# LouisBearing/BirdSoundClassif

Hardware: AMD Instinct MI355X
Metric: clips/sec (3 s @ 22.05 kHz) detect fwd (higher is better)
Workload: dtype f32

## Files before the change

birdsoundclassif_amd/_lib.py:

```python
import ctypes as C
import os
import subprocess

_HERE = os.path.dirname(os.path.abspath(__file__))
LIB_PATH = os.environ.get('NBM_LIB') or os.path.join(_HERE, 'libnbm_hip.so')
CSRC = os.path.join(_HERE, 'csrc')

_lib = None


class GemmDesc(C.Structure):
    _fields_ = [('x', C.c_void_p), ('w', C.c_void_p), ('y', C.c_void_p),
                ('scale', C.c_void_p), ('shift', C.c_void_p), ('residual', C.c_void_p),
                ('x_gs', C.c_int64), ('w_gs', C.c_int64), ('y_gs', C.c_int64), ('res_gs', C.c_int64),
                ('groups', C.c_int),
                ('B', C.c_int), ('H', C.c_int), ('W', C.c_int), ('Cin', C.c_int),
                ('N', C.c_int),
                ('kh', C.c_int), ('kw', C.c_int), ('stride', C.c_int), ('pad', C.c_int),
                ('Ho', C.c_int), ('Wo', C.c_int),
                ('x_ld', C.c_int), ('w_ld', C.c_int), ('y_ld', C.c_int), ('res_ld', C.c_int),
                ('alpha', C.c_float), ('act', C.c_int), ('shift_per_row', C.c_int),
                ('up', C.c_void_p), ('up_H', C.c_int), ('up_W', C.c_int),
                ('rows', C.c_void_p), ('rows_blocks', C.c_void_p),
                ('rows_mode', C.c_int), ('rows_count', C.c_int), ('rows_TH', C.c_int), ('rows_TW', C.c_int),
                ('mask', C.c_void_p), ('mask_ld', C.c_int), ('bits_out', C.c_void_p)]


class RoiDesc(C.Structure):
    _fields_ = [('fmap', C.c_void_p * 5), ('fh', C.c_int * 5), ('fw', C.c_int * 5),
                ('n_levels', C.c_int), ('C', C.c_int),
                ('rois', C.c_void_p), ('n_roi', C.c_void_p), ('B', C.c_int), ('roi_cap', C.c_int),
                ('pe_f', C.c_void_p), ('pe_t', C.c_void_p), ('img_h', C.c_int), ('img_w', C.c_int),
                ('pool', C.c_void_p), ('pe', C.c_void_p), ('level', C.c_void_p), ('n_roi_per_image', C.c_int)]


class AugmentParams(C.Structure):
    _fields_ = [('gain', C.c_float), ('coef', C.c_float), ('denom', C.c_float), ('neg_coef', C.c_float),
                ('neg_denom', C.c_float), ('flags', C.c_int32), ('hard_index', C.c_int32), ('pad', C.c_int32),
                ('noise_seed', C.c_uint64)]


class BwdDesc(C.Structure):
    _fields_ = [('g', C.c_void_p), ('w', C.c_void_p), ('x', C.c_void_p), ('out', C.c_void_p),
                ('a_scale', C.c_void_p), ('row_scale', C.c_void_p), ('residual', C.c_void_p), ('mask', C.c_void_p),
                ('g_gs', C.c_int64), ('w_gs', C.c_int64), ('x_gs', C.c_int64), ('out_gs', C.c_int64), ('res_gs', C.c_int64),
                ('groups', C.c_int),
                ('B', C.c_int), ('H', C.c_int), ('W', C.c_int), ('Cin', C.c_int), ('N', C.c_int),
                ('kh', C.c_int), ('kw', C.c_int), ('stride', C.c_int), ('pad', C.c_int), ('Ho', C.c_int), ('Wo', C.c_int),
                ('g_ld', C.c_int), ('w_ld', C.c_int), ('x_ld', C.c_int), ('out_ld', C.c_int), ('res_ld', C.c_int),
                ('mask_ld', C.c_int), ('alpha', C.c_float), ('bias_grad', C.c_void_p), ('residual2', C.c_void_p), ('res2_ld', C.c_int),
                ('mask_bits', C.c_void_p)]


_P, _I, _L, _F, _U64 = C.c_void_p, C.c_int, C.c_int64, C.c_float, C.c_uint64

SIGNATURES = {
    'nbm_graph_census': [_P, C.POINTER(C.c_longlong * 6)],
    'nbm_copy_rect': [_P, _P, _L, _L, _I, _L, _L, _I, _I, _P],
    'nbm_gemm_conv': [C.POINTER(GemmDesc), _P],
    'nbm_pcm16_to_wave': [_P, _L, _I, _I, _I, _P, _L, _L, _P, _L, _I, _I, _P],
    'nbm_resample_to_wave': [_P, _L, _I, _L, _I, _I, _P, _I, _L, _L, _P, _L, _I, _I, _I, _P],
    'nbm_minmax_init': [_P, _I, _P],
    'nbm_stft_db': [_P, _L, _I, _I, _I, _I, _P, _I, _I, _I, _F, _P, _L, _I, _P, _P],
    'nbm_spec_windows': [_P, _L, _I, _I, _I, _I, _P, _P, _I, _I, _I, _P, _P],
    'nbm_spec_windows_table': [_P, _I, _I, _P, _I, _I, _P],
    'nbm_init_conv': [_P, _L, _P, _P, _I, _P, _P],
    'nbm_stem7x7': [_P, _I, _I, _I, _P, _P, _P, _P, _P, _P, _P],
    'nbm_stem7x7_wgrad': [_P, _P, _I, _I, _I, _P, _P, _P],
    'nbm_maxpool3x3s2': [_P, _I, _I, _I, _I, _P, _I, _I, _P, _P],
    'nbm_space_to_batch2': [_P, _I, _I, _I, _I, _P, _I, _P],
    'nbm_avgpool2x2': [_P, _I, _I, _I, _I, _P, _P],
    'nbm_avgpool2x2_bwd': [_P, _I, _I, _I, _I, _P, _P],
    'nbm_upsample_bilinear_add': [_P, _I, _I, _I, _I, _P, _P, _I, _I, _P],
    'nbm_softmax_rows': [_P, _L, _I, _L, _P],
    'nbm_dwconv3x3': [_P, _I, _I, _I, _I, _I, _I, _P, _P, _P, _L, _P, _I, _I, _P],
    'nbm_silu': [_P, _P, _L, _P],
    'nbm_layernorm': [_P, _L, _I, _P, _P, _F, _P, _P],
    'nbm_mha_small': [_P, _P, _P, _I, _I, _I, _P, _I, _I, _I, _I, _I, _L, _L, _P, _F, _P],
    'nbm_pair_softmax': [_P, _L, _I, _I, _P, _I, _P],
    'nbm_rpn_decode': [_P, _P, _P, _I, _I, _I, _I, _I, _I, _P, _P, _P, _P],
    'nbm_rpn_select': [_P, _P, _P, _I, _I, _I, _I, _I, _P, _P, _P, _I, _P],
    'nbm_nms_batched': [_P, _P, _P, _I, _I, _F, _I, _P, _P, _P, _P, _P, _I, _P],
    'nbm_rpn_select_seg': [_P, _P, _P, _I, _I, _I, _I, _I, _P, _P, _P, _P, _P],
    'nbm_nms_batched_seg': [_P, _P, _P, _I, _I, _F, _I, _P, _P, _P, _P, _P, _P, _P],
    'nbm_roi_pool': [C.POINTER(RoiDesc), _P],
    'nbm_rcnn_post': [_P, _P, _I, _I, _P, _P, _I, _I, _I, _F, _F, _I, _P, _P, _I, _P],
    'nbm_merge_collect': [_P, _P, _I, _I, _I, _I, _I, _L, _P, _P, _P, _P, _P, _P],
    'nbm_merge_nms_workspace': [_I, C.POINTER(C.c_int64)],
    'nbm_merge_nms': [_P, _P, _I, _F, _P, _L, _P, _P, _P],
    'nbm_merge_gather': [_P, _P, _P, _P, _P, _I, _P, _P, _P],
    'nbm_conv_dgrad': [C.POINTER(BwdDesc), _P],
    'nbm_conv_wgrad': [C.POINTER(BwdDesc), _P],
    'nbm_relu_bwd': [_P, _P, _P, _L, _P],
    'nbm_silu_bwd': [_P, _P, _P, _L, _P],
    'nbm_axpby': [_P, _P, _P, _F, _F, _L, _L, _P],
    'nbm_colsum': [_P, _L, _I, _I, _P, _P],
    'nbm_leaky_relu_bwd': [_P, _P, _P, _F, _L, _P],
    'nbm_layernorm_bwd': [_P, _P, _P, _L, _I, _F, _P, _P, _P, _P],
    'nbm_mha_small_bwd': [_P, _P, _P, _P, _I, _I, _I, _I, _P, _P, _P, _I, _I, _I, _P, _I, _I, _I, _I, _L, _L, _P, _F, _P],
    'nbm_zero_roi_windows': [_P, _I, _I, _I, _P, _P, _I, _I, _I, _P],
    'nbm_zero_pattern': [_P, _I, _I, _I, _I, _I, _P],
    'nbm_zero_tiles': [_P, _I, _I, _I, _I, _P, _I, _P, _P],
    'nbm_tiles_gather': [_P, _I, _I, _I, _I, _P, _I, _P, _P, _P],
    'nbm_tiles_scatter_add': [_P, _I, _I, _I, _I, _P, _I, _P, _P, _P],
    'nbm_proposal_iou': [_P, _P, _P, _I, _I, _I, _P, _P, _P],
    'nbm_anchor_targets': [_P, _I, _P, _P, _I, _I, _F, _F, _P, _P, _P, _P],
    'nbm_maxpool3x3s2_bwd': [_P, _P, _P, _I, _I, _I, _I, _I, _I, _P, _P, _P],
    'nbm_upsample_bilinear_bwd': [_P, _I, _I, _I, _I, _P, _I, _I, _I, _P],
    'nbm_tiles_upsample_bilinear_bwd_add': [_P, _I, _I, _I, _I, _P, _I, _P, _P, _I, _I, _P],
    'nbm_png_unfilter_gray8': [_P, _L, _I, _I, _I, _P, _L, _P, _P],
    'nbm_image_half_std_u8': [_P, _L, _I, _L, _P, _P],
    'nbm_randn_fill': [_U64, _L, _P, _P],
    'nbm_augment_batch': [_P, _P, _P, _I, _I, _I, _P, _P, _P, _P, _P, _P, _P],
    'nbm_u8_to_unit': [_P, _L, _P, _P],
    'nbm_wino_input': [_P, _I, _I, _I, _I, _P, _I, _P],
    'nbm_wino_output': [_P, _P, _P, _P, _I, _I, _I, _I, _I, _P, _I, _P, _P],
    'nbm_wino_outgrad': [_P, _I, _I, _I, _I, _P, _P, _I, _P],
    'nbm_wino_weight': [_P, _P, _I, _I, _I, _I, _P, _P],
    'nbm_wino_weight_grad': [_P, _P, _I, _I, _I, _P, _P],
    'nbm_wino23_rows': [_P, _I, _I, _I, _I, _P, _P],
    'nbm_wino23_conv_fused': [_P, _P, _P, _P, _P, _I, _I, _I, _I, _I, _I, _P, _I, _P],
    'nbm_wino23_rows_tiles': [_P, _I, _I, _I, _I, _P, _I, _P, _P, _P, _I, _P],
    'nbm_wino23_conv_fused_tiles': [_P, _P, _P, _P, _P, _I, _I, _I, _I, _I, _I, _P, _P, _I, _P, _P, _P],
    'nbm_roi_tiles': [_P, _P, _I, _I, _I, _I, _P, _P, _P, _I, _P, _P, _I, _P],
    'nbm_wino23_input_tiles': [_P, _I, _I, _I, _I, _P, _I, _P, _P, _P],
    'nbm_wino23_outgrad_tiles': [_P, _I, _I, _I, _I, _P, _I, _P, _P, _P, _I, _P],
    'nbm_cell_outgrad': [_P, _I, _I, _I, _I, _I, _P, _P, _P],
    'nbm_cell_weight': [_P, _I, _I, _P, _I, _P, _I, _P],
    'nbm_cell_weight_fold': [_P, _P, _I, _I, _I, _I, _F, _P, _I, _P, _I, _P],
    'nbm_cell_weight_grad': [_P, _I, _I, _I, _P, _P],
    'nbm_cell_input': [_P, _I, _I, _I, _I, _I, _P, _I, _I, _P],
    'nbm_cell_input_up': [_P, _P, _I, _I, _I, _I, _I, _I, _I, _P, _I, _I, _P],
    'nbm_cell_patches': [_P, _I, _I, _I, _I, _I, _P, _I, _I, _P],
    'nbm_cell_patches_up': [_P, _P, _I, _I, _I, _I, _I, _I, _I, _P, _I, _I, _P],
    'nbm_cell_dgrad_output': [_P, _I, _I, _I, _I, _I, _P, _I, _I, _I, _P, _P],
    'nbm_cell_output': [_P, _P, _I, _I, _I, _I, _I, _P, _P],
    'nbm_weighted_sum': [_P, _P, _P, _P, _P, _L, _P],
    'nbm_weighted_sum_bwd': [_P, _P, _P, _P, _P, _P, _P, _P, _P, _L, _P],
    'nbm_softmax_rows_bwd': [_P, _P, _P, _L, _I, _F, _P],
    'nbm_pair_softmax_bwd': [_P, _P, _P, _L, _P],
    'nbm_dwconv3x3_bwd': [_P, _P, _P, _I, _I, _I, _I, _I, _I, _P, _P, _P, _I, _I, _P],
    'nbm_dwconv3x3_bwd_acc': [_P, _P, _I, _I, _I, _I, _I, _I, _P, _I, _I, _P],
    'nbm_film_fwd': [_P, _P, _P, _L, _I, _P],
    'nbm_film_bwd': [_P, _P, _P, _P, _P, _L, _I, _P],
    'nbm_bn_train_fwd': [_P, _L, _I, _P, _P, _F, _F, _P, _P, _P, _P, _P, _P, _P],
    'nbm_bn_train_bwd': [_P, _P, _L, _I, _P, _P, _P, _P, _P, _P, _P, _P],
    'nbm_roi_pool_bwd': [C.POINTER(C.c_void_p), C.POINTER(C.c_int), C.POINTER(C.c_int), _I, _I, _P, _P, _I, _I, _P, _P],
    'nbm_sqnorm_accum': [_P, _L, _P, _P],
    'nbm_adamw_step': [_P, _P, _P, _P, _L, _F, _F, _F, _F, _F, _I, _P, _F, _P],
}


def build(verbose=False):
    r = subprocess.run(['make', '-C', CSRC, '-j4'], capture_output=True, text=True)
    if verbose or r.returncode:
        print(r.stdout[-4000:], r.stderr[-4000:])
    if r.returncode:
        raise RuntimeError('building libnbm_hip.so failed')
    return LIB_PATH


def load():
    global _lib
    if _lib is not None:
        return _lib
    import torch
    if not os.path.isfile(LIB_PATH):
        raise RuntimeError(f'{LIB_PATH} is missing: build it with `python -c "import __graft_entry__ as g; g.build()"` '
                           '(the NBM hot path has no CPU / eager fallback)')
    lib = C.CDLL(LIB_PATH)
    lib.nbm_version.restype = C.c_char_p
    lib.nbm_version.argtypes = []
    for name, argtypes in SIGNATURES.items():
        fn = getattr(lib, name)
        fn.argtypes = argtypes
        fn.restype = C.c_int
    _lib = lib
    return lib


class NbmHipError(RuntimeError):
    pass


_CODES = {-1: 'NBM_EINVAL (bad argument / shape)', -2: 'NBM_EALIGN (pointer or pitch not 16-byte aligned)',
          -3: 'NBM_EUNSUPPORTED'}


def check(rc, name):
    if rc != 0:
        raise NbmHipError(f'{name} failed: {_CODES.get(rc, f"hipError_t {rc}")}')
```

birdsoundclassif_amd/nets/backbone.py:

```python
import torch
from torch import nn

from .. import ops
from . import _prep, functional as Fn
from .position_encoding import build_position_encoding

bcbk_channels = {'resnet': {'2': 64, '3': 256, '4': 512, '5': 1024, '6': 2048}}
_RESNET_LAYERS = {'resnet50': [3, 4, 6, 3], 'resnet101': [3, 4, 23, 3], 'resnet152': [3, 8, 36, 3]}


class FrozenBatchNorm2d(nn.Module):

    def __init__(self, n):
        super().__init__()
        self.register_buffer('weight', torch.ones(n))
        self.register_buffer('bias', torch.zeros(n))
        self.register_buffer('running_mean', torch.zeros(n))
        self.register_buffer('running_var', torch.ones(n))

    def _load_from_state_dict(self, state_dict, prefix, local_metadata, strict, missing_keys, unexpected_keys,
                              error_msgs):
        state_dict.pop(prefix + 'num_batches_tracked', None)
        super()._load_from_state_dict(state_dict, prefix, local_metadata, strict, missing_keys, unexpected_keys,
                                      error_msgs)

    def affine(self):
        return _prep.bn_affine(self.weight, self.bias, self.running_mean, self.running_var, 1e-5, frozen=True)


class _Bottleneck(nn.Module):

    def __init__(self, inplanes, planes, stride, downsample, norm_layer):
        super().__init__()
        self.conv1 = nn.Conv2d(inplanes, planes, 1, bias=False)
        self.bn1 = norm_layer(planes)
        self.conv2 = nn.Conv2d(planes, planes, 3, stride=stride, padding=1, bias=False)
        self.bn2 = norm_layer(planes)
        self.conv3 = nn.Conv2d(planes, planes * 4, 1, bias=False)
        self.bn3 = norm_layer(planes * 4)
        self.downsample = downsample
        self.stride = stride
        self.mask_input, self.mask_gy = False, True

    def forward(self, x):
        if torch.is_grad_enabled() and x.dim() == 4 and self.conv1.weight.shape[0] % 32 == 0:
            ds = self.downsample
            sd, bd = ds[1].affine() if ds is not None else (None, None)
            return Fn.Bottleneck.apply(x, self.conv1.weight, self.conv2.weight, self.conv3.weight,
                                       ds[0].weight if ds is not None else None, *self.bn1.affine(), *self.bn2.affine(),
                                       *self.bn3.affine(), sd, bd, self.stride, self.mask_input, self.mask_gy)
        s, b = self.bn1.affine()
        o = Fn.conv(x, self.conv1.weight, scale=s, shift=b, act=ops.ACT_RELU)
        s, b = self.bn2.affine()
        if self.stride == 1 and Fn._winograd_ok(o, self.conv2.weight, 3, 3, 1, 1):
            o = ops.conv3x3_winograd(o, _prep.wino23(self.conv2.weight), b, scale=s, relu=True)
        else:
            o = Fn.conv(o, self.conv2.weight, scale=s, shift=b, kh=3, kw=3, stride=self.stride, pad=1, act=ops.ACT_RELU)
        if self.downsample is not None:
            s, b = self.downsample[1].affine()
            idt = Fn.conv(x, self.downsample[0].weight, scale=s, shift=b, stride=self.stride)
        else:
            idt = x
        s, b = self.bn3.affine()
        return Fn.conv(o, self.conv3.weight, scale=s, shift=b, residual=idt, act=ops.ACT_RELU)


class _ResNetBody(nn.Module):

    def __init__(self, layers, norm_layer, dilation=False):
        super().__init__()
        self.conv1 = nn.Conv2d(3, 64, 7, stride=2, padding=3, bias=False)
        self.bn1 = norm_layer(64)
        self.dilation = bool(dilation)
        inplanes = 64
        for li, (planes, n, stride) in enumerate(zip((64, 128, 256, 512), layers, (1, 2, 2, 1 if dilation else 2)), start=1):
            blocks = []
            for bi in range(n):
                st = stride if bi == 0 else 1
                ds = None
                if bi == 0 and (st != 1 or inplanes != planes * 4):
                    ds = nn.Sequential(nn.Conv2d(inplanes, planes * 4, 1, stride=st, bias=False), norm_layer(planes * 4))
                blocks.append(_Bottleneck(inplanes, planes, st, ds, norm_layer))
                if dilation and li == 4 and bi > 0:
                    blocks[-1].conv2.dilation, blocks[-1].conv2.padding = (2, 2), (2, 2)
                blocks[-1].mask_input = not (li == 1 and bi == 0)
                blocks[-1].mask_gy = bi == n - 1
                inplanes = planes * 4
            setattr(self, f'layer{li}', nn.Sequential(*blocks))

    def forward(self, x, init_conv=None):
        s, b = self.bn1.affine()
        if init_conv is not None:
            x = Fn.Stem.apply(x, init_conv.weight, init_conv.bias, self.conv1.weight, s, b)
        else:
            x = Fn.conv(x, self.conv1.weight, scale=s, shift=b, kh=7, kw=7, stride=2, pad=3, act=ops.ACT_RELU)
        taps = [x]
        x = Fn.MaxPool.apply(x, True)
        for li in range(1, 5):
            for bi, blk in enumerate(getattr(self, f'layer{li}')):
                if self.dilation and li == 4 and bi == 1:
                    x = Fn.SpaceToBatch2.apply(x, False)
                x = blk(x)
            if self.dilation and li == 4 and len(self.layer4) > 1:
                x = Fn.SpaceToBatch2.apply(x, True)
            taps.append(x)
        return taps


class BackboneBase(nn.Module):

    def __init__(self, backbone, name, in_channels, train_backbone):
        super().__init__()
        for _, parameter in backbone.named_parameters():
            if not train_backbone:
                parameter.requires_grad_(False)
        self.body = backbone
        self.num_channels = list(bcbk_channels['resnet'].values())
        if in_channels != 3:
            self.init_conv = nn.Conv2d(in_channels, 3, 1)
        self.in_channels = in_channels
        self.strides = [2 ** (i + 1) for i in range(len(self.num_channels))]

    def forward(self, x):
        if hasattr(self, 'init_conv'):
            if self.in_channels != 1:
                raise NotImplementedError('init_conv is implemented for 1 input channel (reference default)')
            return self.body(x, self.init_conv)
        return self.body(x)


class Backbone(BackboneBase):

    def __init__(self, name, in_channels, train_backbone, dilation, norm_layer_name):
        if name not in _RESNET_LAYERS:
            raise ValueError(f'not supported {name}: the accelerated path implements {sorted(_RESNET_LAYERS)}')
        if norm_layer_name != 'frozen_batchnorm':
            raise NotImplementedError('only --norm_layer_backbone frozen_batchnorm (reference default) is implemented')
        super().__init__(_ResNetBody(_RESNET_LAYERS[name], FrozenBatchNorm2d, dilation=dilation), name, in_channels, train_backbone)


class Joiner(nn.Sequential):
    def __init__(self, backbone, position_embedding):
        super().__init__(backbone, position_embedding)

    def forward(self, x):
        return self[0](x), None


def build_backbone(args):
    position_embedding = build_position_encoding(args)
    train_backbone = args.lr_backbone > 0
    backbone = Backbone(args.backbone, args.inpt_channels, train_backbone, args.dilation, args.norm_layer_backbone)
    model = Joiner(backbone, position_embedding)
    model.num_channels = backbone.num_channels
    model.strides = backbone.strides
    setattr(args, 'n_layers', len(backbone.num_channels))
    return model
```

birdsoundclassif_amd/ops.py:

```python
import ctypes as C
import os
import math

import torch

from . import _lib
from ._lib import GemmDesc, RoiDesc, check

ACT_NONE, ACT_RELU, ACT_SILU, ACT_LEAKY = 0, 1, 2, 3

PROFILE = None
FLOPS = None
FLOPS_DEFERRED = []


def flops_total():
    tot = FLOPS[0] + sum(float(c.item()) * f for c, f in FLOPS_DEFERRED)
    FLOPS_DEFERRED.clear()
    return tot


_PROFILE_LABEL = None
PROFILE_ONLY = None


def _prof_all():
    return PROFILE is not None and PROFILE_ONLY is None


def _prof_fused():
    return PROFILE is not None and PROFILE_ONLY in (None, 'fused')


def is_deepk(Cin, N, kh, kw, rows=None):
    return rows is None and N > 64 and Cin % 32 == 0 and kh * kw * Cin > 256



def _stream():
    return C.c_void_p(torch.cuda.current_stream().cuda_stream)


def _ptr(t):
    return C.c_void_p(t.data_ptr()) if t is not None else C.c_void_p(0)


def _chk(t, dtype=torch.float32, name='tensor'):
    if not (isinstance(t, torch.Tensor) and t.is_cuda):
        raise RuntimeError(f'{name}: the NBM HIP path needs CUDA (ROCm) tensors; no CPU fallback exists')
    if t.dtype != dtype:
        raise TypeError(f'{name}: expected {dtype}, got {t.dtype}')
    if not t.is_contiguous():
        raise ValueError(f'{name}: must be contiguous')
    return t


def lib():
    return _lib.load()


def gemm_conv(x, w, y, *, B, H, W, Cin, N, kh=1, kw=1, stride=1, pad=0, Ho=None, Wo=None,
              x_ld=None, w_ld=None, y_ld=None, scale=None, shift=None, residual=None, res_ld=None,
              groups=1, x_gs=0, w_gs=0, y_gs=0, res_gs=0, alpha=1.0, act=ACT_NONE, shift_per_row=False, up=None,
              rows=None, rows_mode=0, rows_count=0, rows_blocks=None, rows_thw=(0, 0), mask=None, mask_ld=None, bits_out=None):
    Ho = (H + 2 * pad - kh) // stride + 1 if Ho is None else Ho
    Wo = (W + 2 * pad - kw) // stride + 1 if Wo is None else Wo
    d = GemmDesc()
    d.x, d.w, d.y = x.data_ptr(), w.data_ptr(), y.data_ptr()
    d.scale = scale.data_ptr() if scale is not None else None
    d.shift = shift.data_ptr() if shift is not None else None
    d.residual = residual.data_ptr() if residual is not None else None
    d.x_gs, d.w_gs, d.y_gs, d.res_gs = x_gs, w_gs, y_gs, res_gs
    d.groups = groups
    d.B, d.H, d.W, d.Cin, d.N = B, H, W, Cin, N
    d.kh, d.kw, d.stride, d.pad, d.Ho, d.Wo = kh, kw, stride, pad, Ho, Wo
    d.x_ld = Cin if x_ld is None else x_ld
    d.w_ld = kh * kw * Cin if w_ld is None else w_ld
    d.y_ld = N if y_ld is None else y_ld
    d.res_ld = (N if res_ld is None else res_ld) if residual is not None else 0
    d.alpha, d.act, d.shift_per_row = float(alpha), int(act), int(bool(shift_per_row))
    if up is not None:
        d.up, d.up_H, d.up_W = _chk(up, name='up').data_ptr(), up.shape[1], up.shape[2]
    if mask is not None:
        d.mask, d.mask_ld = mask.data_ptr(), int(N if mask_ld is None else mask_ld)
    if bits_out is not None:
        assert bits_out.dtype == torch.int32 and bits_out.is_contiguous() and bits_out.numel() * 32 >= B * Ho * Wo * N and N % 32 == 0
        d.bits_out = bits_out.data_ptr()
    if rows is not None:
        d.rows, d.rows_mode, d.rows_count = rows.data_ptr(), int(rows_mode), int(rows_count)
        d.rows_blocks = rows_blocks.data_ptr() if rows_blocks is not None else None
        d.rows_TH, d.rows_TW = rows_thw
    if FLOPS is not None:
        if rows is None:
            FLOPS[0] += 2.0 * B * Ho * Wo * N * kh * kw * Cin * groups
        elif rows_blocks is None:
            FLOPS[0] += 2.0 * rows_count * N * Cin
        else:
            FLOPS_DEFERRED.append((rows_blocks.clone(), 2.0 * 128 * (16 if rows_mode == 2 else 1) * N * Cin))
    if _prof_all() or (PROFILE is not None and PROFILE_ONLY == 'deepk' and is_deepk(Cin, N, kh, kw, rows)):
        ev0, ev1 = torch.cuda.Event(enable_timing=True), torch.cuda.Event(enable_timing=True)
        ev0.record()
        check(lib().nbm_gemm_conv(C.byref(d), _stream()), 'nbm_gemm_conv')
        ev1.record()
        if rows is None:
            PROFILE.append(((Cin, N, kh, H, W, B, groups, stride, _PROFILE_LABEL), ev0, ev1))
        elif rows_blocks is None:
            PROFILE.append(((Cin, N, kh, rows_count, 1, 1, groups, stride, ('rows', H, W)), ev0, ev1))
        else:
            PROFILE.append(((Cin, N, kh, 0, 1, 1, groups, stride, ('rows-rois', H, W)), ev0, ev1))
        return y
    check(lib().nbm_gemm_conv(C.byref(d), _stream()), 'nbm_gemm_conv')
    return y


def conv2d(x, w, kh=1, kw=1, stride=1, pad=0, scale=None, shift=None, residual=None, act=ACT_NONE,
           alpha=1.0, out=None, w_ld=None, up=None, bits_out=None):
    _chk(x, name='x'), _chk(w, name='w')
    B, H, W, Cin = x.shape
    N = w.shape[0]
    Ho = (H + 2 * pad - kh) // stride + 1
    Wo = (W + 2 * pad - kw) // stride + 1
    y = out if out is not None else torch.empty((B, Ho, Wo, N), device=x.device, dtype=torch.float32)
    if residual is not None:
        _chk(residual, name='residual')
        assert residual.shape == y.shape
    gemm_conv(x, w, y, B=B, H=H, W=W, Cin=Cin, N=N, kh=kh, kw=kw, stride=stride, pad=pad, Ho=Ho, Wo=Wo,
              w_ld=w.shape[1] if w_ld is None else w_ld, scale=scale, shift=shift, residual=residual,
              alpha=alpha, act=act, up=up, bits_out=bits_out)
    return y


WINO_CHUNK_BYTES = 24 << 30
_WINO_SCRATCH = {}

LANE = 0


class lane:
    def __init__(self, k):
        self.k = int(k)

    def __enter__(self):
        global LANE
        self.prev, LANE = LANE, self.k

    def __exit__(self, *exc):
        global LANE
        LANE = self.prev


def _wino_scratch(device, n_v, n_m):
    need = n_v + n_m
    key = (device, LANE)
    buf = _WINO_SCRATCH.get(key)
    if buf is None or buf.numel() < need:
        if torch.cuda.is_current_stream_capturing():
            raise RuntimeError('the persistent Winograd scratch would have to grow during a graph capture (the warm-up steps of the '
                               'capture must run the same shapes under the same ops.lane)')
        have = 0 if buf is None else buf.numel()
        _WINO_SCRATCH[key] = buf = None
        size = min(max(need, 2 * have), max(need, WINO_CHUNK_BYTES // 4))
        buf = _WINO_SCRATCH[key] = torch.empty((size,), device=device, dtype=torch.float32)
    return buf[:n_v], buf[n_v:need]


GRAPH_NODE_KINDS = ('kernel', 'memcpy', 'memset', 'host', 'empty', 'other')


def graph_census(raw_graph):
    counts = (C.c_longlong * 6)()
    check(_lib.load().nbm_graph_census(C.c_void_p(int(raw_graph)), C.byref(counts)), 'nbm_graph_census')
    return dict(zip(GRAPH_NODE_KINDS, (int(v) for v in counts)))


def lane_buffers(lanes):
    from . import ondemand
    held = [buf for key, buf in _WINO_SCRATCH.items() if key[1] in lanes and buf is not None]
    for key, bufs in ondemand._ROI_TILE_BUF.items():
        if key[2] in lanes:
            held.extend(bufs)
    return held


def release_lane_scratch(keep=(0,)):
    from . import ondemand
    for key in [k for k in _WINO_SCRATCH if k[1] not in keep]:
        del _WINO_SCRATCH[key]
    for key in [k for k in ondemand._ROI_TILE_BUF if k[2] not in keep]:
        del ondemand._ROI_TILE_BUF[key]


WINO_FUSED_VARIANT = int(os.environ.get('NBM_WINO_FUSED_VARIANT', '0'))


def conv3x3_winograd(x, U, bias=None, m=2, scale=None, relu=False, mask=None, residual=None):
    _chk(x, name='x'), _chk(U, name='U')
    B, H, W, C_ = x.shape
    N = U.shape[1]
    nxi = (m + 2) ** 2
    assert U.shape == (nxi, N, C_) and C_ % 32 == 0 and N % 4 == 0
    y = torch.empty((B, H, W, N), device=x.device, dtype=torch.float32)
    tiles = (-(-H // m)) * (-(-W // m))
    fused = m == 2 and C_ >= 64
    assert residual is None or m == 4, 'residual: F(4x4,3x3) output transform only' 
    if fused:
        per_img = 4 * (-(-H // 2)) * (2 * (-(-W // 2)) + 2) * C_ * 4
    else:
        per_img = nxi * tiles * (C_ + N) * 4
    chunk = max(1, min(B, WINO_CHUNK_BYTES // per_img))
    if fused:
        V, M = _wino_scratch(x.device, chunk * per_img // 4, 0)
    else:
        V, M = _wino_scratch(x.device, nxi * chunk * tiles * C_, nxi * chunk * tiles * N)
    st = _stream()
    if _prof_all():
        ev = (torch.cuda.Event(enable_timing=True), torch.cuda.Event(enable_timing=True))
        ev[0].record()
    for b0 in range(0, B, chunk):
        nb = min(chunk, B - b0)
        T = nb * tiles
        mk = _ptr(mask[b0:b0 + nb]) if mask is not None else None
        if fused:
            check(lib().nbm_wino23_rows(_ptr(x[b0:b0 + nb]), nb, H, W, C_, _ptr(V), st), 'nbm_wino23_rows')
            if FLOPS is not None:
                FLOPS[0] += 2.0 * nxi * T * C_ * N
            if _prof_fused():
                e0, e1 = torch.cuda.Event(enable_timing=True), torch.cuda.Event(enable_timing=True)
                e0.record()
            check(lib().nbm_wino23_conv_fused(_ptr(V), _ptr(U), _ptr(scale), _ptr(bias), mk, int(relu), nb, H, W, C_, N,
                                              _ptr(y[b0:b0 + nb]), WINO_FUSED_VARIANT, st), 'nbm_wino23_conv_fused')
            if _prof_fused():
                e1.record()
                PROFILE.append(((C_, N, 1, T, 1, 1, nxi, 1, ('wino23', H, W)), e0, e1))
            continue
        check(lib().nbm_wino_input(_ptr(x[b0:b0 + nb]), nb, H, W, C_, _ptr(V), m, st), 'nbm_wino_input')
        global _PROFILE_LABEL
        _PROFILE_LABEL = ('wino23', H, W)
        try:
            gemm_conv(V, U, M, B=1, H=T, W=1, Cin=C_, N=N, groups=nxi, x_gs=T * C_, w_gs=N * C_, y_gs=T * N)
        finally:
            _PROFILE_LABEL = None
        check(lib().nbm_wino_output(_ptr(M), _ptr(scale), _ptr(bias), mk, int(relu), nb, H, W, N, _ptr(y[b0:b0 + nb]), m,
                                    _ptr(residual[b0:b0 + nb]) if residual is not None else None, st), 'nbm_wino_output')
    if _prof_all():
        ev[1].record()
        PROFILE.append((('wino23', C_, N, H, W, B), *ev))
    return y


def wino_weight(weight, transposed=False, m=2, scale=None):
    _chk(weight, name='weight')
    N, C_ = weight.shape[:2]
    assert tuple(weight.shape[2:]) == (3, 3)
    No, Co = (C_, N) if transposed else (N, C_)
    U = torch.empty(((m + 2) ** 2, No, Co), device=weight.device, dtype=torch.float32)
    check(lib().nbm_wino_weight(_ptr(weight), _ptr(scale), N, C_, int(bool(transposed)), m, _ptr(U), _stream()),
          'nbm_wino_weight')
    return U


def wino_weight_grad(dU, m=2, row_scale=None):
    _chk(dU, name='dU')
    _, N, C_ = dU.shape
    dW = torch.empty((N, C_, 3, 3), device=dU.device, dtype=torch.float32)
    check(lib().nbm_wino_weight_grad(_ptr(dU), _ptr(row_scale), N, C_, m, _ptr(dW), _stream()), 'nbm_wino_weight_grad')
# ... 844 lines not shown
```

include/nbm_hip.h:

```cpp
#ifndef NBM_HIP_H
#define NBM_HIP_H

#include <stdint.h>

#ifdef __cplusplus
extern "C" {
#endif

#define NBM_OK 0
#define NBM_EINVAL (-1)
#define NBM_EALIGN (-2)
#define NBM_EUNSUPPORTED (-3)

#define NBM_ACT_NONE 0
#define NBM_ACT_RELU 1
#define NBM_ACT_SILU 2
#define NBM_ACT_LEAKY 3

const char* nbm_version(void);

int nbm_graph_census(void* graph, long long counts[6]);

typedef struct nbm_gemm_desc {
  const float* x;
  const float* w;
  float* y;
  const float* scale;
  const float* shift;
  const float* residual;
  int64_t x_gs, w_gs, y_gs, res_gs;
  int groups;
  int B, H, W, Cin;
  int N;
  int kh, kw, stride, pad;
  int Ho, Wo;
  int x_ld, w_ld, y_ld, res_ld;
  float alpha;
  int act;
  int shift_per_row;
  const float* up;
  int up_H, up_W;
  const int* rows;
  const int* rows_blocks;
  int rows_mode, rows_count, rows_TH, rows_TW;
  const float* mask;
  int mask_ld;
  unsigned* bits_out;
} nbm_gemm_desc;

int nbm_gemm_conv(const nbm_gemm_desc* d, void* stream);

int nbm_wino_input(const float* x, int B, int H, int W, int C, float* V, int m, void* stream);
int nbm_wino_output(const float* M, const float* scale, const float* shift, const float* mask, int relu, int B, int H, int W,
                    int N, float* y, int m, const float* residual, void* stream);
int nbm_wino_outgrad(const float* g, int B, int H, int W, int N, float* dM, float* bias_grad, int m, void* stream);

int nbm_wino_weight(const float* g, const float* scale, int N, int C, int transposed, int m, float* U, void* stream);
int nbm_wino_weight_grad(const float* dU, const float* row_scale, int N, int C, int m, float* dW, void* stream);

int nbm_wino23_rows(const float* x, int B, int H, int W, int C, float* R, void* stream);
int nbm_wino23_conv_fused(const float* R, const float* U, const float* scale, const float* shift, const float* mask,
                          int relu, int B, int H, int W, int C, int N, float* y, int variant, void* stream);

int nbm_wino23_rows_tiles(const float* x, int B, int H, int W, int C, const int* tiles, int n_entries, const int* n_blocks,
                          const unsigned* blk_info, float* R,
                          int skip_pattern_stride ,
                          void* stream);
int nbm_wino23_conv_fused_tiles(const float* R, const float* U, const float* scale, const float* shift, const float* mask,
                                int relu ,
                                int B, int H, int W, int C, int N, float* y, const int* tiles, int n_entries,
                                const int* n_blocks, const unsigned* blk_info, void* stream);
int nbm_roi_tiles(const float* rois, const int* n_roi, int B, int roi_cap, int n_levels, int level, const int* fh,
                  const int* fw, const unsigned char* skip, int dilate, int* tiles, int* n_blocks,
                  int per_image , void* stream);
int nbm_wino23_input_tiles(const float* x, int B, int H, int W, int C, const int* tiles, int n_list, const unsigned* plane_mask,
                           float* V, void* stream);
int nbm_wino23_outgrad_tiles(const float* g, int B, int H, int W, int N, const int* tiles, int n_list, const unsigned* plane_mask,
                             float* dM, float* bias_grad, int skip_pattern_stride, void* stream);
int nbm_cell_outgrad(const float* g, int B, int H, int W, int N, int stride, float* Vg, float* bias_grad, void* stream);
int nbm_cell_weight(const float* w, int N, int C, float* U_nc, int ld, float* U_cn, int ldt, void* stream);
int nbm_cell_weight_fold(const float* w, const float* w_lat, int wl_ld, int N, int C, int Cin, float alpha, float* U_nc, int ld,
                         float* U_cn, int ldt, void* stream);
int nbm_cell_weight_grad(const float* dU, int N, int C, int ld, float* dW, void* stream);
int nbm_cell_input(const float* x, int B, int H, int W, int C, int stride, float* Vx, int ld ,
                   int c_off , void* stream);
int nbm_cell_input_up(const float* x1, const float* bias, int B, int H, int W, int C, int Hc, int Wc, int stride, float* Vx, int ld,
                      int c_off, void* stream);
int nbm_cell_patches(const float* x, int B, int H, int W, int C, int stride, float* Vx, int ld, int c_off, void* stream);
int nbm_cell_patches_up(const float* x1, const float* bias, int B, int H, int W, int C, int Hc, int Wc, int stride, float* Vx, int ld,
                        int c_off, void* stream);

int nbm_copy_rect(float* strided, float* packed, int64_t n_outer, int64_t outer_pitch, int n_rows, int64_t row_pitch, int64_t width,
                  int to_strided, int zero_strided, void* stream);
int nbm_cell_dgrad_output(const float* M, int B, int H, int W, int C, int stride, float* gx, int parity_class,
                          int ld , int c_off ,
                          float* bias_grad , void* stream);
int nbm_cell_output(const float* M, const float* bias, int B, int H, int W, int N, int stride, float* y, void* stream);


int nbm_pcm16_to_wave(const int16_t* pcm, int64_t pcm_ld, int batch, int n, int upsample,
                      const int32_t* hq, int64_t first, int64_t count, float* out, int64_t out_ld, int lead,
                      int pad_mode, void* stream);

int nbm_resample_to_wave(const float* x, int64_t x_ld, int batch, int64_t n, int L, int M, const double* taps, int T,
                         int64_t first, int64_t count, float* out, int64_t out_ld, int lead, int pad_mode, int quant16,
                         void* stream);

int nbm_minmax_init(uint32_t* minmax, int batch, void* stream);
int nbm_stft_db(const float* wave, int64_t wave_ld, int batch, int n_frames, int hop, int n_fft,
                const double* basis, int basis_bin_tiles, int basis_ksteps, int n_bins, float floor_amp,
                float* db, int64_t db_bs, int db_ld, uint32_t* minmax, void* stream);

int nbm_spec_windows(const float* db, int64_t db_bs, int db_ld, int batch, int n_bins, int n_frames,
                     const uint32_t* minmax, float* img, int n_img, int w_pix, int hop_img,
                     const int32_t* last_cols, void* stream);

typedef struct nbm_window_entry {
  const float* db;
  const uint32_t* minmax;
  const int32_t* last_cols;
  int32_t db_ld, n_frames, window, n_img;
} nbm_window_entry;

int nbm_spec_windows_table(const nbm_window_entry* table, int batch, int n_bins, float* img, int w_pix, int hop_img,
                           void* stream);


int nbm_init_conv(const float* x, int64_t n_pix, const float* w, const float* b, int C, float* y, void* stream);

int nbm_stem7x7(const float* img, int B, int H, int W, const float* weff, const float* wb, const float* wb_full,
                const float* scale, const float* shift, float* y, void* stream);

int nbm_stem7x7_wgrad(const float* img, const float* g, int B, int H, int W, float* D, float* Cb, void* stream);

int nbm_maxpool3x3s2(const float* x, int B, int H, int W, int C, float* y, int Ho, int Wo, uint8_t* idx, void* stream);
int nbm_space_to_batch2(const float* x, int B, int H, int W, int C, float* y, int inverse, void* stream);
int nbm_avgpool2x2(const float* x, int B, int Ho, int Wo, int C, float* y, void* stream);
int nbm_avgpool2x2_bwd(const float* gy, int B, int Ho, int Wo, int C, float* gx, void* stream);

int nbm_upsample_bilinear_add(const float* src, int B, int Hi, int Wi, int C, const float* add,
                              float* y, int Ho, int Wo, void* stream);

int nbm_softmax_rows(float* x, int64_t rows, int cols, int64_t ld, void* stream);

int nbm_dwconv3x3(const float* x, int B, int H, int W, int Cin, int mult, int stride,
                  const float* w , const float* bias, const float* film, int64_t film_ld,
                  float* y, int Ho, int Wo, void* stream);

int nbm_silu(const float* x, float* y, int64_t n, void* stream);

int nbm_layernorm(const float* x, int64_t rows, int E, const float* w, const float* b, float eps, float* y, void* stream);

int nbm_mha_small(const float* q, const float* k, const float* v, int q_ld, int k_ld, int v_ld, float* out, int out_ld,
                  int S, int N, int nhead, int hd, int64_t seq_stride, int64_t batch_stride, const int32_t* n_valid,
                  float scale, void* stream);

int nbm_pair_softmax(const float* x, int64_t n_pix, int n_anchor, int x_ld, float* y, int y_ld, void* stream);


int nbm_rpn_decode(const float* cls, const float* reg, const float* anchors , int B, int KA,
                   int n_anchor , int img_w, int img_h, int min_size, float* boxes,
                   uint32_t* keys, int* keep_count, void* stream);

int nbm_rpn_select(const float* boxes, const uint32_t* keys, const int* keep_count, int B, int KA,
                   int top_n, int fail_below, int cap, float* sel_boxes, float* sel_scores, int* n_sel,
                   int per_image, void* stream);

int nbm_rpn_select_seg(const float* boxes, const uint32_t* keys, const int* keep_count, int B, int KA,
                       int top_n, int fail_below, int cap, float* sel_boxes, float* sel_scores, int* n_sel,
                       const int* seg, void* stream);

int nbm_nms_batched(const float* boxes, const float* scores, const int* n_in, int B, int cap, float thresh,
                    int post_n, uint64_t* mask_ws, int* keep_ws, float* rois, float* roi_scores, int* n_out,
                    int per_image, void* stream);

int nbm_nms_batched_seg(const float* boxes, const float* scores, const int* n_in, int B, int cap, float thresh,
                        int post_n, uint64_t* mask_ws, int* keep_ws, float* rois, float* roi_scores, int* n_out,
                        const int* seg, void* stream);

typedef struct nbm_roi_desc {
  const float* fmap[5];
  int fh[5], fw[5];
  int n_levels, C;
  const float* rois;
  const int* n_roi;
  int B, roi_cap;
  const float* pe_f; const float* pe_t; int img_h, img_w;
  float* pool; float* pe; int* level;
  int n_roi_per_image;
} nbm_roi_desc;
int nbm_roi_pool(const nbm_roi_desc* d, void* stream);

int nbm_rcnn_post(const float* rois, const int* n_roi, int B, int roi_cap, const float* bbox_reg,
                  const float* bbox_cls, int n_cls1 , int img_w, int img_h,
                  float nms_thresh, float min_score, int proposal_number, float* det, int* n_det,
                  int per_image , void* stream);

#define NBM_MERGE_MAX_N 131072

int nbm_merge_collect(const float* det, const int* n_det, int n_img, int cap, int num_classes, int w_pix, int hop,
                      int64_t spectrogram_length, int* cell_ws, float* boxes, float* scores, int* species, int* n_out,
                      void* stream);

// ... 111 lines not shown
```

Baseline: 1082.

## Fuse ResNet layer1 bottleneck tails with downsample and next conv1 in one kernel

Adds a HIP kernel that computes a bottleneck's conv3 1x1 GEMM with BN, residual and ReLU. In the first block it also computes the downsample projection in the same pass. In later blocks it instead chains straight into the next block's conv1 1x1 GEMM with BN and ReLU, keeping the 256-channel output in registers. Layer1 inference now uses this fused path, which removes separate launches and the round-trip re-read of the 256-channel activation, at the cost of a special-cased path tied to fixed channel shapes.

Result: no change. 1089, median of 6 (+0.7%).

```diff
diff --git a/birdsoundclassif_amd/_lib.py b/birdsoundclassif_amd/_lib.py
--- a/birdsoundclassif_amd/_lib.py
+++ b/birdsoundclassif_amd/_lib.py
@@ -58,6 +58,7 @@
     'nbm_graph_census': [_P, C.POINTER(C.c_longlong * 6)],
     'nbm_copy_rect': [_P, _P, _L, _L, _I, _L, _L, _I, _I, _P],
     'nbm_gemm_conv': [C.POINTER(GemmDesc), _P],
+    'nbm_bottleneck_tail': [_P, _P, _P, _P, _P, _P, _P, _P, _P, _P, _P, _P, _P, _I, _P],
     'nbm_pcm16_to_wave': [_P, _L, _I, _I, _I, _P, _L, _L, _P, _L, _I, _I, _P],
     'nbm_resample_to_wave': [_P, _L, _I, _L, _I, _I, _P, _I, _L, _L, _P, _L, _I, _I, _I, _P],
     'nbm_minmax_init': [_P, _I, _P],
diff --git a/birdsoundclassif_amd/csrc/bottleneck_tail.hip b/birdsoundclassif_amd/csrc/bottleneck_tail.hip
--- /dev/null
+++ b/birdsoundclassif_amd/csrc/bottleneck_tail.hip
@@ -0,0 +1,193 @@
+#include "nbm_common.h"
+
+namespace {
+
+constexpr int TK = 64;
+constexpr int TN = 256;
+constexpr int TN1 = 64;
+constexpr int WP3 = TK + 4;
+constexpr int WP1 = TN + 4;
+constexpr int TWAVES = 8;
+
+struct TailParams {
+  const float* a2; const float* w3; const float* s3; const float* b3;
+  const float* x; const float* wd; const float* sd; const float* bd;
+  float* y;
+  const float* w1; const float* s1; const float* b1; float* a1;
+  int M, m_tiles;
+};
+
+__device__ __forceinline__ int perm32(int r) { return 16 * ((r >> 2) & 1) + (r & 3) + 4 * (r >> 3); }
+
+template <bool DS, bool CHAIN>
+__global__ __launch_bounds__(TWAVES * 64, 1) void bottleneck_tail_kernel(const TailParams p) {
+  static_assert(DS != CHAIN, "one of the two seams per launch (LDS budget)");
+  constexpr int W2F = DS ? TN * WP3 : TN1 * WP1;
+  constexpr int VF = DS ? 4 * TN : 2 * TN + 2 * TN1;
+  __shared__ __attribute__((aligned(16))) float lds[TN * WP3 + W2F + VF];
+  float* W3s = lds;
+  float* W2s = lds + TN * WP3;
+  float* V = W2s + W2F;
+  const int tid = threadIdx.x, lane = tid & 63, wave = tid >> 6, li = lane & 31, lh = lane >> 5;
+
+  for (int i = tid; i < TN * (TK / 4); i += TWAVES * 64) {
+    const int r = i / (TK / 4), c = i - r * (TK / 4), src = (r & ~31) | perm32(r & 31);
+    *reinterpret_cast<f32x4*>(W3s + r * WP3 + c * 4) = *reinterpret_cast<const f32x4*>(p.w3 + src * TK + c * 4);
+    if constexpr (DS) *reinterpret_cast<f32x4*>(W2s + r * WP3 + c * 4) = *reinterpret_cast<const f32x4*>(p.wd + src * TK + c * 4);
+  }
+  if constexpr (CHAIN) {
+    for (int i = tid; i < TN1 * (TN / 4); i += TWAVES * 64) {
+      const int r = i / (TN / 4), c = i - r * (TN / 4), src = (r & ~31) | perm32(r & 31);
+      *reinterpret_cast<f32x4*>(W2s + r * WP1 + c * 4) = *reinterpret_cast<const f32x4*>(p.w1 + src * TN + c * 4);
+    }
+  }
+  for (int i = tid; i < TN; i += TWAVES * 64) {
+    V[i] = p.s3[i];
+    V[TN + i] = p.b3[i];
+    if constexpr (DS) { V[2 * TN + i] = p.sd[i]; V[3 * TN + i] = p.bd[i]; }
+    if constexpr (CHAIN) if (i < TN1) { V[2 * TN + i] = p.s1[i]; V[2 * TN + TN1 + i] = p.b1[i]; }
+  }
+  __syncthreads();
+
+  f32x4 a[2][4], an[2][4], xa[DS ? 2 : 1][4], xn[DS ? 2 : 1][4];
+  auto load_rows = [&](const float* base, int tile, f32x4 (*dst)[4]) {
+    int m = tile * 32 + li;
+    m = m < p.M ? m : p.M - 1;
+    const float* rp = base + (long long)m * TK + 16 * lh;
+#pragma unroll
+    for (int kc = 0; kc < 2; ++kc)
+#pragma unroll
+      for (int q = 0; q < 4; ++q) dst[kc][q] = *reinterpret_cast<const f32x4*>(rp + kc * 32 + 4 * q);
+  };
+  auto gemm64 = [&](const float* Ws, int r0, f32x4 (*act)[4]) {
+    f32x16 acc;
+#pragma unroll
+    for (int e = 0; e < 16; ++e) acc[e] = 0.f;
+    const float* wb = Ws + (r0 + li) * WP3 + 16 * lh;
+#pragma unroll
+    for (int kc = 0; kc < 2; ++kc) {
+      f32x4 w[4];
+#pragma unroll
+      for (int q = 0; q < 4; ++q) w[q] = *reinterpret_cast<const f32x4*>(wb + kc * 32 + 4 * q);
+#pragma unroll
+      for (int q = 0; q < 4; ++q)
+#pragma unroll
+        for (int e = 0; e < 4; ++e) acc = __builtin_amdgcn_mfma_f32_32x32x2f32(w[q][e], act[kc][q][e], acc, 0, 0, 0);
+    }
+    return acc;
+  };
+
+  const int step = gridDim.x * TWAVES;
+  int tile = blockIdx.x * TWAVES + wave;
+  if (tile < p.m_tiles) {
+    load_rows(p.a2, tile, an);
+    if constexpr (DS) load_rows(p.x, tile, xn);
+  }
+  for (; tile < p.m_tiles; tile += step) {
+    const int nt = tile + step < p.m_tiles ? tile + step : tile;
+#pragma unroll
+    for (int kc = 0; kc < 2; ++kc)
+#pragma unroll
+      for (int q = 0; q < 4; ++q) {
+        a[kc][q] = an[kc][q];
+        if constexpr (DS) xa[kc][q] = xn[kc][q];
+      }
+    load_rows(p.a2, nt, an);
+    if constexpr (DS) load_rows(p.x, nt, xn);
+    const int m = tile * 32 + li;
+    const bool ok = m < p.M;
+    const long long mc = ok ? m : p.M - 1;
+    f32x4 rq[4], rn[4];
+    auto load_res = [&](int jj, f32x4* dst) {
+#pragma unroll
+      for (int q = 0; q < 4; ++q) dst[q] = *reinterpret_cast<const f32x4*>(p.x + mc * TN + jj * 32 + 16 * lh + 4 * q);
+    };
+    if constexpr (CHAIN) load_res(0, rn);
+    f32x16 acc1[2];
+#pragma unroll
+    for (int j = 0; j < 2; ++j)
+#pragma unroll
+      for (int e = 0; e < 16; ++e) acc1[j][e] = 0.f;
+#pragma unroll 1
+    for (int jj = 0; jj < TN / 32; ++jj) {
+      if constexpr (CHAIN) {
+#pragma unroll
+        for (int q = 0; q < 4; ++q) rq[q] = rn[q];
+        load_res(jj + 1 < TN / 32 ? jj + 1 : jj, rn);
+      }
+      const f32x16 acc = gemm64(W3s, jj * 32, a);
+      f32x16 accd;
+      if constexpr (DS) accd = gemm64(W2s, jj * 32, xa);
+      f32x4 yv[4];
+      const int c0 = jj * 32 + 16 * lh;
+#pragma unroll
+      for (int q = 0; q < 4; ++q) {
+        const f32x4 sc = *reinterpret_cast<const f32x4*>(V + c0 + 4 * q), sh = *reinterpret_cast<const f32x4*>(V + TN + c0 + 4 * q);
+        f32x4 r;
+        if constexpr (DS) {
+          const f32x4 scd = *reinterpret_cast<const f32x4*>(V + 2 * TN + c0 + 4 * q), shd = *reinterpret_cast<const f32x4*>(V + 3 * TN + c0 + 4 * q);
+#pragma unroll
+          for (int e = 0; e < 4; ++e) r[e] = (accd[4 * q + e] * 1.0f) * scd[e] + shd[e] + 0.f;
+        } else {
+          r = rq[q];
+        }
+        f32x4 v;
+#pragma unroll
+        for (int e = 0; e < 4; ++e) v[e] = (acc[4 * q + e] * 1.0f) * sc[e] + sh[e] + 0.f;
+        v[0] += r[0]; v[1] += r[1]; v[2] += r[2]; v[3] += r[3];
+#pragma unroll
+        for (int e = 0; e < 4; ++e) v[e] = fmaxf(v[e], 0.0f);
+        yv[q] = v;
+        if (ok) *reinterpret_cast<f32x4*>(p.y + (long long)m * TN + c0 + 4 * q) = v;
+      }
+      if constexpr (CHAIN) {
+#pragma unroll
+        for (int j = 0; j < 2; ++j) {
+          const float* wb = W2s + (j * 32 + li) * WP1 + jj * 32 + 16 * lh;
+          f32x4 w[4];
+#pragma unroll
+          for (int q = 0; q < 4; ++q) w[q] = *reinterpret_cast<const f32x4*>(wb + 4 * q);
+#pragma unroll
+          for (int q = 0; q < 4; ++q)
+#pragma unroll
+            for (int e = 0; e < 4; ++e) acc1[j] = __builtin_amdgcn_mfma_f32_32x32x2f32(w[q][e], yv[q][e], acc1[j], 0, 0, 0);
+        }
+      }
+    }
+    if constexpr (CHAIN) {
+#pragma unroll
+      for (int j = 0; j < 2; ++j) {
+        const int c0 = j * 32 + 16 * lh;
+#pragma unroll
+        for (int q = 0; q < 4; ++q) {
+          const f32x4 sc = *reinterpret_cast<const f32x4*>(V + 2 * TN + c0 + 4 * q), sh = *reinterpret_cast<const f32x4*>(V + 2 * TN + TN1 + c0 + 4 * q);
+          f32x4 v;
+#pragma unroll
+          for (int e = 0; e < 4; ++e) v[e] = fmaxf((acc1[j][4 * q + e] * 1.0f) * sc[e] + sh[e] + 0.f, 0.0f);
+          if (ok) *reinterpret_cast<f32x4*>(p.a1 + (long long)m * TN1 + c0 + 4 * q) = v;
+        }
+      }
+    }
+  }
+}
+
+}
+
+extern "C" int nbm_bottleneck_tail(const float* a2, const float* w3, const float* s3, const float* b3, const float* x, const float* wd,
+                                   const float* sd, const float* bd, float* y, const float* w1, const float* s1, const float* b1, float* a1,
+                                   int M, void* stream) {
+  if (!a2 || !w3 || !s3 || !b3 || !x || !y || M <= 0) return NBM_EINVAL;
+  const bool ds = wd != nullptr, chain = w1 != nullptr;
+  if (ds == chain) return NBM_EUNSUPPORTED;
+  if (ds && (!sd || !bd)) return NBM_EINVAL;
+  if (chain && (!s1 || !b1 || !a1)) return NBM_EINVAL;
+  const void* ptrs[] = {a2, w3, s3, b3, x, wd, sd, bd, y, w1, s1, b1, a1};
+  for (const void* q : ptrs)
+    if (q && !nbm_aligned16(q)) return NBM_EALIGN;
+  TailParams p{a2, w3, s3, b3, x, wd, sd, bd, y, w1, s1, b1, a1, M, (M + 31) / 32};
+  const int wgs = (p.m_tiles + TWAVES - 1) / TWAVES, gx = wgs < 256 ? wgs : 256;
+  hipStream_t st = (hipStream_t)stream;
+  if (ds) hipLaunchKernelGGL((bottleneck_tail_kernel<true, false>), dim3(gx), dim3(TWAVES * 64), 0, st, p);
+  else hipLaunchKernelGGL((bottleneck_tail_kernel<false, true>), dim3(gx), dim3(TWAVES * 64), 0, st, p);
+  return nbm_launch_status();
+}
diff --git a/birdsoundclassif_amd/nets/backbone.py b/birdsoundclassif_amd/nets/backbone.py
--- a/birdsoundclassif_amd/nets/backbone.py
+++ b/birdsoundclassif_amd/nets/backbone.py
@@ -50,12 +50,7 @@
                                        ds[0].weight if ds is not None else None, *self.bn1.affine(), *self.bn2.affine(),
                                        *self.bn3.affine(), sd, bd, self.stride, self.mask_input, self.mask_gy)
         s, b = self.bn1.affine()
-        o = Fn.conv(x, self.conv1.weight, scale=s, shift=b, act=ops.ACT_RELU)
-        s, b = self.bn2.affine()
-        if self.stride == 1 and Fn._winograd_ok(o, self.conv2.weight, 3, 3, 1, 1):
-            o = ops.conv3x3_winograd(o, _prep.wino23(self.conv2.weight), b, scale=s, relu=True)
-        else:
-            o = Fn.conv(o, self.conv2.weight, scale=s, shift=b, kh=3, kw=3, stride=self.stride, pad=1, act=ops.ACT_RELU)
+        o = self._conv2(Fn.conv(x, self.conv1.weight, scale=s, shift=b, act=ops.ACT_RELU))
         if self.downsample is not None:
             s, b = self.downsample[1].affine()
             idt = Fn.conv(x, self.downsample[0].weight, scale=s, shift=b, stride=self.stride)
@@ -63,6 +58,42 @@
             idt = x
         s, b = self.bn3.affine()
         return Fn.conv(o, self.conv3.weight, scale=s, shift=b, residual=idt, act=ops.ACT_RELU)
+
+    def _conv2(self, o):
+        s, b = self.bn2.affine()
+        if self.stride == 1 and Fn._winograd_ok(o, self.conv2.weight, 3, 3, 1, 1):
+            o = ops.conv3x3_winograd(o, _prep.wino23(self.conv2.weight), b, scale=s, relu=True)
+        else:
+            o = Fn.conv(o, self.conv2.weight, scale=s, shift=b, kh=3, kw=3, stride=self.stride, pad=1, act=ops.ACT_RELU)
+        return o
+
+
+def _layer1_seams_ok(blocks, x):
+    b0 = blocks[0]
+    return (not torch.is_grad_enabled() and x.dim() == 4 and x.shape[-1] == 64 and x.is_contiguous() and x.dtype == torch.float32
+            and b0.downsample is not None and b0.stride == 1 and tuple(b0.downsample[0].weight.shape) == (256, 64, 1, 1)
+            and all(tuple(b.conv1.weight.shape[:2]) == (64, 256 if i else 64) and tuple(b.conv3.weight.shape) == (256, 64, 1, 1)
+                    and b.stride == 1 and (i == 0 or b.downsample is None) for i, b in enumerate(blocks)))
+
+
+def _layer1_seams(blocks, x):
+    a1 = None
+    for i, blk in enumerate(blocks):
+        if a1 is None:
+            s, b = blk.bn1.affine()
+            a1 = Fn.conv(x, blk.conv1.weight, scale=s, shift=b, act=ops.ACT_RELU)
+        o = blk._conv2(a1)
+        s3, b3 = blk.bn3.affine()
+        w3 = _prep.krsc(blk.conv3.weight)
+        if i == 0:
+            sd, bd = blk.downsample[1].affine()
+            x, a1 = ops.bottleneck_tail(o, w3, s3, b3, x=x, wd=_prep.krsc(blk.downsample[0].weight), sd=sd, bd=bd), None
+        elif i + 1 < len(blocks):
+            s1, b1 = blocks[i + 1].bn1.affine()
+            x, a1 = ops.bottleneck_tail(o, w3, s3, b3, residual=x, w1=_prep.krsc(blocks[i + 1].conv1.weight), s1=s1, b1=b1)
+        else:
+            x = Fn.conv(o, blk.conv3.weight, scale=s3, shift=b3, residual=x, act=ops.ACT_RELU)
+    return x
 
 
 class _ResNetBody(nn.Module):
@@ -97,6 +128,10 @@
         taps = [x]
         x = Fn.MaxPool.apply(x, True)
         for li in range(1, 5):
+            if li == 1 and _layer1_seams_ok(self.layer1, x):
+                x = _layer1_seams(self.layer1, x)
+                taps.append(x)
+                continue
             for bi, blk in enumerate(getattr(self, f'layer{li}')):
                 if self.dilation and li == 4 and bi == 1:
                     x = Fn.SpaceToBatch2.apply(x, False)
diff --git a/birdsoundclassif_amd/ops.py b/birdsoundclassif_amd/ops.py
--- a/birdsoundclassif_amd/ops.py
+++ b/birdsoundclassif_amd/ops.py
@@ -111,6 +111,36 @@
         return y
     check(lib().nbm_gemm_conv(C.byref(d), _stream()), 'nbm_gemm_conv')
     return y
+
+
+def bottleneck_tail(a2, w3, s3, b3, *, x=None, wd=None, sd=None, bd=None, residual=None, w1=None, s1=None, b1=None, out=None, out_a1=None):
+    B, H, W, K = _chk(a2, name='a2').shape
+    assert K == 64 and tuple(w3.shape) == (256, 64) and (wd is None) != (w1 is None)
+    M = B * H * W
+    y = torch.empty((B, H, W, 256), device=a2.device, dtype=torch.float32) if out is None else _chk(out, name='out')
+    assert y.shape == (B, H, W, 256)
+    a1 = None
+    if wd is not None:
+        assert tuple(wd.shape) == (256, 64) and tuple(x.shape) == (B, H, W, 64)
+        src = _chk(x, name='x')
+    else:
+        assert tuple(w1.shape) == (64, 256) and tuple(residual.shape) == (B, H, W, 256)
+        src = _chk(residual, name='residual')
+        a1 = torch.empty((B, H, W, 64), device=a2.device, dtype=torch.float32) if out_a1 is None else _chk(out_a1, name='out_a1')
+        assert a1.shape == (B, H, W, 64)
+    if FLOPS is not None:
+        FLOPS[0] += 2.0 * M * 256 * 64 * 2
+    args = (_ptr(a2), _ptr(_chk(w3)), _ptr(_chk(s3)), _ptr(_chk(b3)), _ptr(src), _ptr(wd), _ptr(sd), _ptr(bd), _ptr(y),
+            _ptr(w1), _ptr(s1), _ptr(b1), _ptr(a1), M, _stream())
+    if _prof_all():
+        ev0, ev1 = torch.cuda.Event(enable_timing=True), torch.cuda.Event(enable_timing=True)
+        ev0.record()
+        check(lib().nbm_bottleneck_tail(*args), 'nbm_bottleneck_tail')
+        ev1.record()
+        PROFILE.append(((64, 256, 1, H, W, B, 1, 1, ('tail-ds' if wd is not None else 'tail-chain', H, W)), ev0, ev1))
+    else:
+        check(lib().nbm_bottleneck_tail(*args), 'nbm_bottleneck_tail')
+    return y if a1 is None else (y, a1)
 
 
 def conv2d(x, w, kh=1, kw=1, stride=1, pad=0, scale=None, shift=None, residual=None, act=ACT_NONE,
diff --git a/include/nbm_hip.h b/include/nbm_hip.h
--- a/include/nbm_hip.h
+++ b/include/nbm_hip.h
@@ -49,6 +49,10 @@
 } nbm_gemm_desc;
 
 int nbm_gemm_conv(const nbm_gemm_desc* d, void* stream);
+
+int nbm_bottleneck_tail(const float* a2, const float* w3, const float* s3, const float* b3, const float* x, const float* wd,
+                        const float* sd, const float* bd, float* y, const float* w1, const float* s1, const float* b1, float* a1,
+                        int M, void* stream);
 
 int nbm_wino_input(const float* x, int B, int H, int W, int C, float* V, int m, void* stream);
 int nbm_wino_output(const float* M, const float* scale, const float* shift, const float* mask, int relu, int B, int H, int W,
```
